# weitianxin/MACR

Hardware: AMD Instinct MI355X
Metric: train interactions/sec + eval users/sec (full-catalog top-K@20) (higher is better)
Workload: dtype f32; 1 GPU; gowalla-shape MACR-MF rubibceboth d=64 batch=4096 c=40 (n_users=29858, n_items=40981); synthetic Xavier tables, Zipf positives, batches as sampled (grouped on the device inside the step); parallelism=replicas x1 (train) / item-sharded x1 + RCCL all-gather (eval), global_batch=4096

## Files before the change

### macr_amd/csrc/train_kernels.hip

```cpp
#include "common.hpp"
#include "refsort.hpp"
#include "spmm.hpp"

#include <type_traits>

namespace macr {

#ifdef MACR_ABL_NOATOMIC
#define MACR_ATOMIC_ADD(p, v) (*(p) = (v))
#else
#define MACR_ATOMIC_ADD(p, v) unsafeAtomicAdd((p), (v))
#endif

constexpr int kPartStride = 4;

template <int LPR>
struct RowGroup {
    static constexpr int kRowsPerWave = kWave / LPR;
    static constexpr int kRowsPerBlock = 256 / LPR;
    int sub;
    int slot;
    __device__ RowGroup() {
        sub = threadIdx.x % LPR;
        slot = threadIdx.x / LPR;
// ... 383 lines not shown
    __shared__ float s_lr[kLazyRing];
    s_lr[threadIdx.x] = state->lr[threadIdx.x];
    const uint32_t T = state->t;
    __syncthreads();
    const int sub = threadIdx.x % LPR;
    for (long long k = blockIdx.x * (256LL / LPR) + threadIdx.x / LPR; k < n; k += gridDim.x * (256LL / LPR)) {
        const int row = rows[k];
        float4 x = make_float4(0, 0, 0, 0);
        if (row >= 0) x = lazy_row4<LPR>(tb, row, sub, T, s_lr, b1, b2, eps);
        st4(out + ((size_t)k * LPR + sub) * 4, x);
    }
}

constexpr float kBxbYHi = 6.0f, kBxbYLoPairs = -60.0f, kBxbYLoSingle = -20.0f;
constexpr float kBprZLoPairs = -40.0f;
constexpr int kNeutralTileMax = 8;

struct PendingAdam {
    const float *mU, *vU, *gU, *mI, *vI, *gI;
    int32_t *tU, *tI;
    const float *mw, *vw, *mwu, *vwu;
    const StepScalars *scal;
    float b1, b2, eps;
    const uint32_t *stU, *stI;
    const LazyState *lazy;
};

template <int LPR, int PENDING, bool RUBIBPR = false>
__global__ __launch_bounds__(256) void k_pair_fwd(
    int B, int Bp, const int32_t *__restrict__ u, const int32_t *__restrict__ i, const int32_t *__restrict__ j,
    const float *__restrict__ Usrc, const float *__restrict__ Isrc,
    const float *__restrict__ w, const float *__restrict__ wu,
    float *__restrict__ fwd, float *__restrict__ part, int reg_on_gathered, float *__restrict__ gw, PendingAdam pa,
    int user_branch, const float *__restrict__ Bsrc = nullptr) {
    constexpr int d = 4 * LPR;
    __shared__ float red[48];
    __shared__ float s_lr[PENDING == 2 ? kLazyRing : 1];
    RowGroup<LPR> g;
    const int t = blockIdx.x * RowGroup<LPR>::kRowsPerBlock + g.slot;
    float sq = 0.f, litem = 0.f, luser = 0.f;
    uint32_t T = 0;
    if (PENDING == 2) {
        s_lr[threadIdx.x] = pa.lazy->lr[threadIdx.x];
        T = pa.lazy->t;
        __syncthreads();
    }
    if (!PENDING && blockIdx.x == 0) {
        for (int k = threadIdx.x; k < kBranchSlots * 2 * d; k += 256) gw[k] = 0.f;
    }
    if (t < B) {
        const int ru = u[t], ri = i[t], rj = j[t];
        float4 eu = ld4(Usrc + (size_t)ru * d + 4 * g.sub);
        float4 ei = ld4(Isrc + (size_t)ri * d + 4 * g.sub);
        float4 ej = ld4(Isrc + (size_t)rj * d + 4 * g.sub);
        float4 w4 = ld4(w + 4 * g.sub), wu4 = ld4(wu + 4 * g.sub);
        if (PENDING) {
            const float lr_t = pa.scal->lr_t;
            const size_t au = (size_t)ru * d + 4 * g.sub, ai = (size_t)ri * d + 4 * g.sub, aj = (size_t)rj * d + 4 * g.sub;
            float4 mu = ld4(pa.mU + au), vu = ld4(pa.vU + au), mi = ld4(pa.mI + ai), vi = ld4(pa.vI + ai);
            float4 mj = ld4(pa.mI + aj), vj = ld4(pa.vI + aj);
            const float4 gu = ld4(pa.gU + au), gi = ld4(pa.gI + ai), gj = ld4(pa.gI + aj);
            float4 gw4 = make_float4(0, 0, 0, 0), gwu4 = make_float4(0, 0, 0, 0);
#pragma unroll
            for (int k = 0; k < kBranchSlots; ++k) {
                gw4 = add4(gw4, ld4(gw + (size_t)k * 2 * d + 4 * g.sub));
                gwu4 = add4(gwu4, ld4(gw + (size_t)k * 2 * d + d + 4 * g.sub));
            }
            float4 mw4 = ld4(pa.mw + 4 * g.sub), vw4 = ld4(pa.vw + 4 * g.sub);
            float4 mwu4 = ld4(pa.mwu + 4 * g.sub), vwu4 = ld4(pa.vwu + 4 * g.sub);
            if (PENDING == 2) {
                const uint32_t upto = T - 1u, su_ = pa.stU[ru], si_ = pa.stI[ri], sj_ = pa.stI[rj];
                if (g.sub == 0) {
// ... 31 lines not shown
            const float ssi = sigmoid_acc(si), ssj = sigmoid_acc(sj), ssu = user_branch ? sigmoid_acc(su) : 1.0f;
            fwd[0 * (size_t)Bp + t] = p;
            fwd[1 * (size_t)Bp + t] = n;
            fwd[2 * (size_t)Bp + t] = ssi * ssu;
            fwd[3 * (size_t)Bp + t] = ssj * ssu;
            fwd[4 * (size_t)Bp + t] = ssi;
            fwd[5 * (size_t)Bp + t] = ssj;
            if (RUBIBPR) {
                float hi, hj;
                litem = PairLossBPR::term(si, sj, 1.0f, hi, hj);
                fwd[6 * (size_t)Bp + t] = fabsf(hj);
            } else {
                fwd[6 * (size_t)Bp + t] = (p < -20.0f || n > kBxbYHi || n < kBxbYLoPairs) ? -ssu : ssu;
                litem = -logf(ssi + eps) + -logf((1.0f - ssj) + eps);
            }
            luser = user_branch ? -logf(ssu + eps) + -logf((1.0f - ssu) + eps) : 0.0f;
        }
    }
    float s0 = sq, s1 = litem, s2 = luser;
    block_sum3(s0, s1, s2, red);
    if (threadIdx.x == 0) {
        float *o = part + (size_t)blockIdx.x * kPartStride;
        o[0] = s0; o[1] = s1; o[2] = s2; o[3] = 0.f;
    }
}

struct BatchSort {
    const int32_t *u, *i, *j;
    int B;
    int rb0;
    int32_t *perm, *us, *is, *js;
    const float *outflag;
    int nneu, ncbx;
};

constexpr int kBucketSpan = 512;

template <int NW>
__device__ __forceinline__ void batch_bucket_block(const BatchSort &s, int part, uint32_t *s_hist ) {
    const int t = threadIdx.x, wid = t >> 6, lane = t & 63;
    const int plo = part * kBucketSpan, phi = plo + kBucketSpan < s.B ? plo + kBucketSpan : s.B;
    constexpr int per = kBucketSpan / NW;
    const int lo = plo + wid * per < phi ? plo + wid * per : phi, hi = lo + per < phi ? lo + per : phi;
    const uint32_t *keys = reinterpret_cast<const uint32_t *>(s.i);
    for (int k = t; k < NW * kRadix; k += NW * 64) s_hist[k] = 0;
    __syncthreads();
    wave_count(keys, lo, hi, 0, s_hist + wid * kRadix);
    __syncthreads();
    block_digit_offsets<NW>(s_hist, s_hist + NW * kRadix, nullptr, 0);
    uint32_t *offs = s_hist + wid * kRadix;
    const uint64_t below = (1ull << lane) - 1ull;
    constexpr int NQ = per / 64;
    int32_t ri[NQ], ru[NQ], rj[NQ];
    if (lo < hi) {
#pragma unroll
        for (int q = 0; q < NQ; ++q) {
            const int p = lo + q * 64 + lane, pc = p < hi ? p : hi - 1;
            ri[q] = s.i[pc]; ru[q] = s.u[pc]; rj[q] = s.j[pc];
        }
    }
#pragma unroll
    for (int q = 0; q < NQ; ++q) {
        if (lo + q * 64 >= hi) break;
        const int p = lo + q * 64 + lane;
        const bool valid = p < hi;
        const uint32_t dgt = (uint32_t)ri[q] & 255u;
// ... 54 lines not shown
                const float4 f4 = at < B ? ld4(sort.outflag + at + 4 * e) : make_float4(0, 0, 0, 0);
                bits |= ((__float_as_uint(f4.x) >> 31) | ((__float_as_uint(f4.y) >> 31) << 1) | ((__float_as_uint(f4.z) >> 31) << 2) |
                         ((__float_as_uint(f4.w) >> 31) << 3)) << (4 * e);
            }
            int mine = __popc(bits);
            const int pair2 = mine + __shfl_xor(mine, 1, 64);
            const int tile = pair2 + __shfl_xor(pair2, 2, 64);
            if (tile > kNeutralTileMax) mine = 0;
            for (uint64_t hit = __ballot(mine != 0); hit; hit &= hit - 1) {
                const int src = __builtin_ctzll(hit);
                for (uint32_t wv = (uint32_t)__builtin_amdgcn_readlane((int)bits, src); wv; wv &= wv - 1) {
                    const int mine_now = idx++ % nslot == slot;
                    if (!mine_now) continue;
                    const int cj = base + 16 * src + __builtin_ctz(wv);
                    const v2f pn = {p[cj], n[cj]};
                    v2f accj = {0.f, 0.f};
#pragma unroll
                    for (int q = 0; q < R; ++q) {
                        const v2f z = pn * (abn[q] * (-kLog2e));
                        const v2f dd = v2f{__builtin_amdgcn_exp2f(z.x), __builtin_amdgcn_exp2f(z.y)} + one;
                        const v2f sg = {__builtin_amdgcn_rcpf(dd.x), __builtin_amdgcn_rcpf(dd.y)};
                        const v2f om = one - sg;
                        const v2f ts = sg + eps, tom = om + eps;
                        const float txy = ts.x * tom.y;
                        l2n += __builtin_amdgcn_logf(txy);
                        const float r2 = __builtin_amdgcn_rcpf(txy);
                        const v2f h = (sg * om) * r2;
                        const v2f g = v2f{h.x * tom.y, h.y * ts.x};
                        dabn[q] = __builtin_elementwise_fma(g, pn, dabn[q]);
                        accj = __builtin_elementwise_fma(g, abn[q], accj);
                    }
                    const float sx = wave_sum(accj.x), sy = wave_sum(accj.y);
                    if (lane == 0) {
                        colpart[((size_t)rb * 2 + 0) * Bp + cj] = -sx;
                        colpart[((size_t)rb * 2 + 1) * Bp + cj] = sy;
                    }
                }
            }
        }
#pragma unroll
        for (int q = 0; q < R; ++q) {
            s_row[wid][0][q * 64 + lane] = -dabn[q].x;
            s_row[wid][1][q * 64 + lane] = dabn[q].y;
        }
        const float lsum = block_sum(-l2n * kLn2, red);
        if (t == 0) lpart[(size_t)rb * ncbx + ncb + part] = lsum;
        for (int e = t; e < 2 * RB; e += 256) {
            const int q = e / RB, rr = e % RB, r = rb * RB + rr;
            rowpart[((size_t)(ncb + part) * 2 + q) * Bp + r] = (s_row[0][q][rr] + s_row[1][q][rr]) + (s_row[2][q][rr] + s_row[3][q][rr]);
        }
        return;
    }
    if ((int)blockIdx.x >= nbxb + nbn && (int)blockIdx.x < nbxb + nbn + nsort) {
        __builtin_amdgcn_s_setprio(3);
#ifndef MACR_ABL_NOGROUP
        batch_bucket_block<4>(sort, blockIdx.x - nbxb - nbn, s_hist);
#endif
        return;
    }
    const bool is_adam = ADAM && (int)blockIdx.x >= nbxb + nbn + nsort;
    const int ablk = blockIdx.x - nbxb - nbn - nsort, bblk = blockIdx.x;
    if (is_adam) {
#ifndef MACR_ABL_ADAM_NOPRIO
        __builtin_amdgcn_s_setprio(3);
#endif
        if (ADAM == 2) adam_lazy_scan_block(adam, (long long)ablk, scal->lr_t, s_red);
        else adam_block<true>(adam, (long long)ablk, scal->lr_t, s_red);
        return;
    }
    const int cb = bblk % ncb, rb = sort.rb0 + bblk / ncb, t = threadIdx.x, lane = t & 63, wid = t >> 6;
    const float *p = fwd, *n = fwd + Bp, *a = fwd + 2 * (size_t)Bp, *b = fwd + 3 * (size_t)Bp;
    const float kLog2e = 1.4426950408889634f, kLn2 = 0.6931471805599453f;
    const v2f one = {1.0f, 1.0f}, eps = {1e-10f, 1e-10f};
    v2f ab[R], abs_[R], dab[R];
    bool rok[R];
#pragma unroll
    for (int q = 0; q < R; ++q) {
        const int r = rb * RB + q * 64 + lane;
        rok[q] = FULL || r < B;
        ab[q] = v2f{rok[q] ? a[r] : 0.f, rok[q] ? b[r] : 0.f};
        abs_[q] = ab[q] * (-kLog2e);
        dab[q] = v2f{0.f, 0.f};
// ... 180 lines not shown
#if defined(MACR_ABL_BXB_EXACT)
    const bool fast = false;
#elif defined(MACR_ABL_BXB_FORCEFAST)
    const bool fast = true;
#else
    float amax = 0.f, bmax = 0.f;
#pragma unroll
    for (int q = 0; q < R; ++q) { amax = fmaxf(amax, ab[q].x); bmax = fmaxf(bmax, ab[q].y); }
#pragma unroll
    for (int m = 1; m < 64; m <<= 1) { amax = fmaxf(amax, __shfl_xor(amax, m, 64)); bmax = fmaxf(bmax, __shfl_xor(bmax, m, 64)); }
    constexpr float YLO = R >= 2 ? kBxbYLoPairs : kBxbYLoSingle, YHI = kBxbYHi;
    const float xlo = cn.x * amax, yv = cn.y * bmax;
    bool out;
    if constexpr (CELL == kCellBpr) {
        bool nan_row = false;
#pragma unroll
        for (int q = 0; q < R; ++q) nan_row = nan_row || !(ab[q].x + ab[q].y == ab[q].x + ab[q].y);
        out = nan_row || !(fminf(xlo, 0.f) - fmaxf(yv, 0.f) >= kBprZLoPairs) || !(cn.x == cn.x) || !(cn.y == cn.y);
    } else {
        out = !(xlo >= -20.0f) || !(yv >= YLO) || !(yv <= YHI) || !(amax <= 1.0f) || !(bmax <= 1.0f);
    }
    const bool fast = !__any(out);
#endif
    if constexpr (CELL == kCellBpr) {
        if constexpr (R == 1) run_tile_bpr(std::true_type{});
        else if (fast) run_tile_bpr(std::true_type{});
        else run_tile_bpr(std::false_type{});
    } else if (fast) {
        if constexpr (R >= 2) run_tile_pairs(); else run_tile(std::true_type{});
    } else {
        run_tile(std::false_type{});
    }
    if (FULL && sort.nneu) l2.x += 2.0f * (float)(R * (int)__popcll(__ballot(own_out)));
    if (cok && !own_out) {
        colpart[((size_t)rb * 2 + 0) * Bp + c] = -acc.x;
        colpart[((size_t)rb * 2 + 1) * Bp + c] = acc.y;
    }
#pragma unroll
    for (int q = 0; q < R; ++q) {
        s_row[wid][0][q * 64 + lane] = -dab[q].x;
        s_row[wid][1][q * 64 + lane] = dab[q].y;
    }
    const float lsum = block_sum(-(l2.x + l2.y) * kLn2, red);
    if (t == 0) lpart[(size_t)rb * ncbx + cb] = lsum;
    for (int e = t; e < 2 * RB; e += 256) {
        const int q = e / RB, rr = e % RB, r = rb * RB + rr;
        if (FULL || r < B)
            rowpart[((size_t)cb * 2 + q) * Bp + r] = (s_row[0][q][rr] + s_row[1][q][rr]) + (s_row[2][q][rr] + s_row[3][q][rr]);
    }
}

constexpr int kChunkT = 16;

template <int D>
struct WaveRow {
    static constexpr int EPL = (D + 63) / 64;
    static constexpr int kActive = D < 64 ? D : 64;
};

template <int D, bool EGO = false>
__device__ __forceinline__ void combine_positive_rows(const int *s_pos, const float (*s_gi)[D], float *gI,
                                                      int32_t *cnt = nullptr, const float *s_sb = nullptr, float *sbr = nullptr) {
    constexpr int NP = D >= 256 ? 1 : 256 / D;
    const int k = threadIdx.x % D, part = threadIdx.x / D;
    int rows[kChunkT];
#pragma unroll
    for (int s = 0; s < kChunkT; ++s) rows[s] = s_pos[s];
#pragma unroll
    for (int L = 0; L < kChunkT; ++L) {
        if (rows[L] < 0 || (L % NP) != part) continue;
        bool first = true;
#pragma unroll
        for (int s0 = 0; s0 < L; ++s0) first = first && rows[s0] != rows[L];
        if (!first) continue;
        float acc = s_gi[L][k], sb = EGO ? s_sb[L] : 0.f;
        int mult = 1;
#pragma unroll
        for (int s2 = L + 1; s2 < kChunkT; ++s2)
            if (rows[s2] == rows[L]) { acc += s_gi[s2][k]; ++mult; if (EGO) sb += s_sb[s2]; }
        MACR_ATOMIC_ADD(gI + (size_t)rows[L] * D + k, acc);
        if (cnt && k == 0) atomicAdd(cnt + rows[L], mult);
        if (EGO && k == 0) MACR_ATOMIC_ADD(sbr + rows[L], sb);
    }
}

template <int D, bool EGO = false, bool RUBIBPR = false>
__global__ __launch_bounds__(256) void k_pair_bwd(
    int B, int Bp, int nrb, int ncb, const int32_t *__restrict__ perm, const int32_t *__restrict__ u,
    const int32_t *__restrict__ i, const int32_t *__restrict__ j, const float *__restrict__ Usrc,
    const float *__restrict__ Isrc,
    const float *__restrict__ w, const float *__restrict__ wu, const float *__restrict__ fwd,
    const float *__restrict__ rowpart, const float *__restrict__ colpart,
    float *gU, float *gI, int32_t *touchedU, int32_t *touchedI, float *__restrict__ wpart,
    float alpha, float beta, float coef, float *adam_pow, StepScalars *scal, float lr, float b1, float b2,
    LossArgs L, int32_t *cnt_pos, LazyState *lazy = nullptr, int nneu = 0, const float *__restrict__ Bsrc = nullptr,
    float *sbr = nullptr) {
    constexpr int EPL = WaveRow<D>::EPL;
    __shared__ float s_w[4][2][D];
    __shared__ float s_gi[kChunkT][D];
    __shared__ int s_pos[kChunkT];
    __shared__ float s_sb[EGO ? kChunkT : 1];
    const int nblk = gridDim.x - 1;
    if ((int)blockIdx.x == nblk) {
        if (threadIdx.x == 0) {
            const float p1 = adam_pow[0], p2 = adam_pow[1];
            const float lr_t = lr * sqrtf(1.0f - p2) / (1.0f - p1);
            scal->lr_t = lr_t;
            adam_pow[0] = p1 * b1;
            adam_pow[1] = p2 * b2;
            if (lazy) lazy_tick(lazy, lr_t);
        }
        if (L.losses && threadIdx.x < 64) finalize_losses(L, threadIdx.x);
        return;
    }
    const int lane = threadIdx.x & 63, wid = threadIdx.x >> 6;
    const bool act = lane < WaveRow<D>::kActive;
    float wk[EPL], wuk[EPL], aw[EPL], awu[EPL];
#pragma unroll
    for (int e = 0; e < EPL; ++e) {
        const int k = lane + 64 * e;
        wk[e] = act ? w[k] : 0.f; wuk[e] = act ? wu[k] : 0.f; aw[e] = 0.f; awu[e] = 0.f;
    }
    const float inv_b2 = 1.0f / ((float)B * (float)B), eps = 1e-10f, invB = 1.0f / (float)B;
    constexpr int SPW = kChunkT / 4;
    for (int chunk = blockIdx.x; chunk * kChunkT < B; chunk += nblk) {
        const int slot0 = chunk * kChunkT + wid * SPW;
        int my_idx = 0;
        {
            const int tq = slot0 + (lane % SPW);
            if (lane < 4 * SPW && tq < B) my_idx = (lane < SPW ? u : lane < 2 * SPW ? i : lane < 3 * SPW ? j : perm)[tq];
        }
        float reu[SPW][EPL], rei[SPW][EPL], rej[SPW][EPL];
        float rbi[EGO ? SPW : 1][EPL], rbj[EGO ? SPW : 1][EPL];
        int rru[SPW], rri[SPW], rrj[SPW];
#pragma unroll
        for (int q = 0; q < SPW; ++q) {
            rru[q] = __shfl(my_idx, q, kWave); rri[q] = __shfl(my_idx, SPW + q, kWave); rrj[q] = __shfl(my_idx, 2 * SPW + q, kWave);
#pragma unroll
            for (int e = 0; e < EPL; ++e) {
                const int k = act ? lane + 64 * e : 0;
                reu[q][e] = Usrc[(size_t)rru[q] * D + k]; rei[q][e] = Isrc[(size_t)rri[q] * D + k]; rej[q][e] = Isrc[(size_t)rrj[q] * D + k];
                if (EGO) { rbi[q][e] = Bsrc[(size_t)rri[q] * D + k]; rbj[q][e] = Bsrc[(size_t)rrj[q] * D + k]; }
            }
        }
        const int q_own = lane >> 4, kk = lane & 15;
        float dp = 0.f, dn = 0.f, da = 0.f, db = 0.f, ssi = 0.f, ssj = 0.f, ssu = 0.f;
        const bool own_ok = slot0 + q_own < B;
        const int t_own = own_ok ? __shfl(my_idx, 3 * SPW + q_own, kWave) : 0;
        {
            float cp[4], cn[4], ra[2], rb[2];
#pragma unroll
            for (int m = 0; m < 4; ++m) {
                const int k = kk + 16 * m, kc = k < nrb ? k : 0;
                cp[m] = colpart[((size_t)kc * 2) * Bp + t_own]; cn[m] = colpart[((size_t)kc * 2 + 1) * Bp + t_own];
            }
#pragma unroll
            for (int m = 0; m < 2; ++m) {
                const int k = kk + 16 * m, kc = k < ncb ? k : 0;
                ra[m] = rowpart[((size_t)kc * 2) * Bp + t_own]; rb[m] = rowpart[((size_t)kc * 2 + 1) * Bp + t_own];
            }
            const int kn = kk < nneu ? ncb + kk : 0;
            const float dan = rowpart[((size_t)kn * 2) * Bp + t_own], dbn = rowpart[((size_t)kn * 2 + 1) * Bp + t_own];
            const float sg = fabsf(fwd[(4 + (kk < 3 ? kk : 0)) * (size_t)Bp + t_own]);
#pragma unroll
            for (int m = 0; m < 4; ++m) { const bool ok = own_ok && kk + 16 * m < nrb; dp += ok ? cp[m] : 0.f; dn += ok ? cn[m] : 0.f; }
#pragma unroll
            for (int m = 0; m < 2; ++m) { const bool ok = own_ok && kk + 16 * m < ncb; da += ok ? ra[m] : 0.f; db += ok ? rb[m] : 0.f; }
            const bool neu_ok = own_ok && kk < nneu;
            da += neu_ok ? dan : 0.f; db += neu_ok ? dbn : 0.f;
            ssi = (own_ok && kk < 3) ? sg : 0.f;
            if (own_ok) {
                for (int k = kk + 64; k < nrb; k += 16) { dp += colpart[((size_t)k * 2) * Bp + t_own]; dn += colpart[((size_t)k * 2 + 1) * Bp + t_own]; }
                for (int k = kk + 32; k < ncb; k += 16) { da += rowpart[((size_t)k * 2) * Bp + t_own]; db += rowpart[((size_t)k * 2 + 1) * Bp + t_own]; }
            }
        }
#pragma unroll
        for (int m = 1; m < 16; m <<= 1) {
            dp += __shfl_xor(dp, m, kWave); dn += __shfl_xor(dn, m, kWave);
            da += __shfl_xor(da, m, kWave); db += __shfl_xor(db, m, kWave);
        }
        ssj = __shfl(ssi, (lane & 48) + 1, kWave); ssu = __shfl(ssi, (lane & 48) + 2, kWave); ssi = __shfl(ssi, lane & 48, kWave);
        dp *= inv_b2; dn *= inv_b2; da *= inv_b2; db *= inv_b2;
        const float hbpr = ssu;
        if (RUBIBPR) ssu = 1.0f;
        const float dsi_own = da * (ssi * (1.0f - ssi)) * ssu + (alpha * invB) * (RUBIBPR ? -hbpr : dneglog_sig(ssi, eps));
        const float dsj_own = db * (ssj * (1.0f - ssj)) * ssu + (alpha * invB) * (RUBIBPR ? hbpr : dneglog_1msig(ssj, eps));
        const float dsu_own = (da * ssi + db * ssj) * (ssu * (1.0f - ssu)) +
                              (beta * invB) * (dneglog_sig(ssu, eps) + dneglog_1msig(ssu, eps));
#pragma unroll
        for (int q = 0; q < SPW; ++q) {
            const int slot = wid * SPW + q;
            if (slot0 + q >= B) { if (lane == 0) s_pos[slot] = -1; continue; }
            const float dpq = __shfl(dp, q * 16, kWave), dnq = __shfl(dn, q * 16, kWave);
            const float dsi = __shfl(dsi_own, q * 16, kWave), dsj = __shfl(dsj_own, q * 16, kWave), dsu = __shfl(dsu_own, q * 16, kWave);
            const int ru = rru[q], ri = rri[q], rj = rrj[q];
            if (act) {
#pragma unroll
                for (int e = 0; e < EPL; ++e) {
                    const int k = lane + 64 * e;
                    const float eu = reu[q][e], ei = rei[q][e], ej = rej[q][e];
                    const float gu = fmaf(coef, eu, fmaf(dsu, wuk[e], fmaf(dnq, ej, dpq * ei)));
                    const float gi = EGO ? fmaf(coef, ei, dpq * eu) : fmaf(coef, ei, fmaf(dsi, wk[e], dpq * eu));
                    const float gj = EGO ? fmaf(coef, ej, dnq * eu) : fmaf(coef, ej, fmaf(dsj, wk[e], dnq * eu));
                    MACR_ATOMIC_ADD(gU + (size_t)ru * D + k, gu);
                    MACR_ATOMIC_ADD(gI + (size_t)rj * D + k, gj);
                    s_gi[slot][k] = gi;
                    if (EGO) aw[e] = fmaf(dsi, rbi[EGO ? q : 0][e], fmaf(dsj, rbj[EGO ? q : 0][e], aw[e]));
                    else aw[e] = fmaf(dsi, ei, fmaf(dsj, ej, aw[e]));
                    awu[e] = fmaf(dsu, eu, awu[e]);
                }
            }
            if (lane == 0) {
// ... 662 lines not shown
#ifdef MACR_BXB_ROWS
    return MACR_BXB_ROWS;
#endif
    static const int forced = getenv("MACR_BXB_ROWS") ? atoi(getenv("MACR_BXB_ROWS")) : 0;
    if (forced == 1 || forced == 2 || forced == 4) return forced;
    if (B >= 4096) return 4;
    return 1;
}

static inline bool use_staging(int B) {
    static const char *env = getenv("MACR_STAGING");
    if (env && (env[0] == '0' || env[0] == '1')) return env[0] == '1';
    return B > kSmallBatchMax;
}

struct PairWs {
    StepScalars *scal;
    float *gw;
    bool staged;
    int32_t *perm, *us, *is, *js;
    uint32_t *ska, *sva, *skb, *svb;
    uint32_t *ghist;
    uint32_t *n_work;
    float *stage;
    int nblk_bwd;
    float *fwd;
    float *part;
    float *part2;
    float *lpart;
    float *rowpart;
    float *colpart;
    int Bp, nrb, ncb, rows, nblk_pair;
    int nneu, ncbx;
    float *cpart;
    float *wblk;
    float *spart;
    size_t bytes;
};

static PairWs carve_pair_ws(void *base, int B, int d, bool force_staged = false, bool neutral = true) {
    PairWs w;
    const int lpr = d / 4, rpb = 256 / lpr;
    w.Bp = (int)align_up((size_t)B, 256);
    w.rows = bxb_rows(B);
    w.nrb = w.Bp / (64 * w.rows);
    w.ncb = w.Bp / 256;
    static const bool no_neutral = getenv("MACR_BXB_NEUTRAL") && getenv("MACR_BXB_NEUTRAL")[0] == '0';
    w.nneu = (!force_staged && B % 256 == 0 && !no_neutral && neutral) ? 1 : 0;
    w.ncbx = w.ncb + w.nneu;
    w.nblk_pair = (B + rpb - 1) / rpb;
    w.staged = force_staged || use_staging(B);
    if (w.staged) w.nblk_bwd = w.nblk_pair < 4096 ? w.nblk_pair : 4096;
    else w.nblk_bwd = (B + kChunkT - 1) / kChunkT < 1024 ? (B + kChunkT - 1) / kChunkT : 1024;
    char *p = static_cast<char *>(base);
    size_t off = 0;
    auto take = [&](size_t bytes) { void *r = p ? p + off : nullptr; off += align_up(bytes, 256); return r; };
    w.scal = static_cast<StepScalars *>(take(sizeof(StepScalars)));
    w.gw = static_cast<float *>(take((size_t)kBranchSlots * 2 * d * 4));
    w.fwd = static_cast<float *>(take((size_t)7 * w.Bp * 4));
    const int nblk_loss = (B + kChunkT - 1) / kChunkT < 1024 ? (B + kChunkT - 1) / kChunkT : 1024;
    int npart = w.nblk_pair > w.nblk_bwd ? w.nblk_pair : w.nblk_bwd;
    npart = npart > nblk_loss ? npart : nblk_loss;
    w.part = static_cast<float *>(take((size_t)npart * kPartStride * 4));
    w.part2 = static_cast<float *>(take((size_t)npart * kPartStride * 4));
    w.lpart = static_cast<float *>(take((size_t)w.nrb * w.ncbx * 4));
    w.rowpart = static_cast<float *>(take((size_t)w.ncbx * 2 * w.Bp * 4));
    w.colpart = static_cast<float *>(take((size_t)w.nrb * 2 * w.Bp * 4));
    const size_t nsort = 3 * (size_t)B;
    w.ska = w.sva = w.skb = w.svb = nullptr;
    w.perm = w.us = w.is = w.js = nullptr; w.ghist = nullptr; w.stage = nullptr; w.n_work = nullptr;
    w.cpart = w.wblk = w.spart = nullptr;
    if (w.staged) {
        w.ska = static_cast<uint32_t *>(take(nsort * 4)); w.sva = static_cast<uint32_t *>(take(nsort * 4));
        w.skb = static_cast<uint32_t *>(take(nsort * 4)); w.svb = static_cast<uint32_t *>(take(nsort * 4));
        w.ghist = static_cast<uint32_t *>(take(sort_hist_words((int)nsort) * 4));
        w.n_work = static_cast<uint32_t *>(take(4));
        w.stage = static_cast<float *>(take(nsort * d * 4));
    } else {
        w.perm = static_cast<int32_t *>(take((size_t)B * 4)); w.us = static_cast<int32_t *>(take((size_t)B * 4));
        w.is = static_cast<int32_t *>(take((size_t)B * 4));   w.js = static_cast<int32_t *>(take((size_t)B * 4));
    }
    w.bytes = off;
    return w;
}

static PairWs carve_pair_ws_det(void *base, int B, int d) {
    PairWs w = carve_pair_ws(base, B, d, true, false);
    const int ch = d / 4 < 16 ? d / 4 : 16;
    char *p = static_cast<char *>(base);
    auto take = [&](size_t bytes) { void *r = p ? p + w.bytes : nullptr; w.bytes += align_up(bytes, 256); return r; };
    w.cpart = static_cast<float *>(take(2 * ((3 * (size_t)B + ch - 1) / ch) * d * 4));
    w.wblk = static_cast<float *>(take((size_t)w.nblk_bwd * 2 * d * 4));
    return w;
}

template <int CELL = kCellBce>
static void launch_bxb_rows(const PairWs &ws, int B, int nbxb, const AdamArgs *pending, long long n_adam_blocks,
                            const BatchSort &sort, hipStream_t st) {
    const int nsort = (sort.B + kBucketSpan - 1) / kBucketSpan + sort.nneu * ws.nrb;
    const bool full = B % 256 == 0;
#ifdef MACR_ABL_XNOADAM
    n_adam_blocks = 0;
#endif
    auto launch = [&](auto rows) {
        constexpr int R = decltype(rows)::value;
        if (pending && pending->lazy) {
            const unsigned grid = (unsigned)(nbxb + nsort + n_adam_blocks);
            if (full) k_bxb<R, true, 2, CELL><<<grid, 256, 0, st>>>(B, ws.Bp, ws.ncb, nbxb, ws.fwd, ws.rowpart, ws.colpart, ws.lpart, *pending, ws.scal, sort);
            else      k_bxb<R, false, 2, CELL><<<grid, 256, 0, st>>>(B, ws.Bp, ws.ncb, nbxb, ws.fwd, ws.rowpart, ws.colpart, ws.lpart, *pending, ws.scal, sort);
        } else if (pending) {
            const unsigned grid = (unsigned)(nbxb + nsort + n_adam_blocks);
            if (full) k_bxb<R, true, 1, CELL><<<grid, 256, 0, st>>>(B, ws.Bp, ws.ncb, nbxb, ws.fwd, ws.rowpart, ws.colpart, ws.lpart, *pending, ws.scal, sort);
            else      k_bxb<R, false, 1, CELL><<<grid, 256, 0, st>>>(B, ws.Bp, ws.ncb, nbxb, ws.fwd, ws.rowpart, ws.colpart, ws.lpart, *pending, ws.scal, sort);
        } else {
            AdamArgs none;
            none.n_seg = 0;
            if (full) k_bxb<R, true, 0, CELL><<<nbxb + nsort, 256, 0, st>>>(B, ws.Bp, ws.ncb, nbxb, ws.fwd, ws.rowpart, ws.colpart, ws.lpart, none, ws.scal, sort);
            else      k_bxb<R, false, 0, CELL><<<nbxb + nsort, 256, 0, st>>>(B, ws.Bp, ws.ncb, nbxb, ws.fwd, ws.rowpart, ws.colpart, ws.lpart, none, ws.scal, sort);
        }
    };
    switch (ws.rows) {
        case 1: launch(std::integral_constant<int, 1>()); break;
        case 2: launch(std::integral_constant<int, 2>()); break;
        default: launch(std::integral_constant<int, 4>()); break;
    }
}

static BatchSort batch_sort_args(const PairWs &ws, int B = 0, const int32_t *u = nullptr, const int32_t *i = nullptr,
                                 const int32_t *j = nullptr) {
    BatchSort s;
    s.u = u; s.i = i; s.j = j; s.B = B; s.rb0 = 0;
    s.perm = ws.perm; s.us = ws.us; s.is = ws.is; s.js = ws.js;
    s.outflag = nullptr; s.nneu = 0; s.ncbx = ws.ncb;
    return s;
}

struct RefSort { const uint32_t *sk, *sv; uint32_t *free_key, *free_val; };
static RefSort ref_sort_result(const PairWs &ws, int flip) {
    RefSort r;
    r.sk = flip ? ws.skb : ws.ska; r.sv = flip ? ws.svb : ws.sva;
    r.free_key = flip ? ws.ska : ws.skb; r.free_val = flip ? ws.sva : ws.svb;
    return r;
}
static RefSort launch_ref_sort(int B, int n_urows, int n_irows, const int32_t *u, const int32_t *i, const int32_t *j,
                               const PairWs &ws, hipStream_t st) {
    k_refs_init<<<(B + 255) / 256 < 2048 ? (B + 255) / 256 : 2048, 256, 0, st>>>(B, n_urows, u, i, j, ws.ska, ws.sva, ws.n_work);
    return ref_sort_result(ws, launch_radix_sort(ws.ska, ws.sva, ws.skb, ws.svb, 3 * B, (uint32_t)(n_urows + n_irows - 1), ws.ghist, st));
}
__global__ __launch_bounds__(256) void k_ref_place(int n, const uint32_t *__restrict__ sv, uint32_t *__restrict__ place) {
    for (int p = blockIdx.x * 256 + threadIdx.x; p < n; p += gridDim.x * 256) place[sv[p]] = (uint32_t)p;
}
static int launch_seg_index(int B, int d, int n_urows, int n_irows, const RefSort &r, bool listed, float *gU, float *gI,
                            int32_t *tU, int32_t *tI, const PairWs &ws, hipStream_t st) {
    const int n = 3 * B;
    k_seg_scan<<<(n + 255) / 256, 256, 0, st>>>(n, n_urows, (uint32_t)(n_urows + n_irows), r.sk, tU, tI, r.free_key, ws.n_work);
    MACR_CHECK_LAUNCH("seg_index", st);
    MACR_DISPATCH_LPR(d, (k_seg_sum<LPR><<<1024, 256, 0, st>>>(r.free_key, ws.n_work, n_urows, r.sk, listed ? nullptr : r.sv, ws.stage, gU, gI)));
    MACR_CHECK_LAUNCH("seg_sum", st);
    return MACR_OK;
}
static int launch_seg_reduce(int B, int d, int n_urows, int n_irows, const RefSort &r, float *gU, float *gI, int32_t *tU,
                             int32_t *tI, const float *sst, float *sbr, const PairWs &ws, hipStream_t st) {
    const int n = 3 * B;
    MACR_DISPATCH_LPR(d, (k_seg_reduce<LPR><<<(n + 256 / LPR - 1) / (256 / LPR), 256, 0, st>>>(
                             n, n_urows, (uint32_t)(n_urows + n_irows), r.sk, r.sv, ws.stage, gU, gI, tU, tI, sst, sbr)));
    MACR_CHECK_LAUNCH("seg_reduce", st);
// ... 29 lines not shown
                                  hipStream_t st) {
    const int B = c.B, d = c.d, n_urows = c.n_urows, n_irows = c.n_irows, n = 3 * B;
    float *sbr = sst ? c.sbr : nullptr;
    const RefSort r = launch_ref_sort(B, n_urows, n_irows, c.u, c.i, c.j, ws, st);
    MACR_CHECK_LAUNCH("ref_sort", st);
    if (c.sk_sorted) *c.sk_sorted = r.sk;
    if (sv_sorted) {
        *sv_sorted = r.sv;
        return launch_seg_index(B, d, n_urows, n_irows, r, false, c.gU, c.gI, c.tU, c.tI, ws, st);
    }
    if (ws.cpart) {
        MACR_REQUIRE(!sst || (sbr && ws.spart), MACR_E_UNSUPPORTED, "pair: this workspace has no slots for the ego branch scalars");
        MACR_DISPATCH_LPR(d, (k_seg_reduce<LPR, true><<<(n + 256 / LPR - 1) / (256 / LPR), 256, 0, st>>>(
                                 n, n_urows, (uint32_t)(n_urows + n_irows), r.sk, r.sv, ws.stage, c.gU, c.gI, c.tU, c.tI, sst, sbr, ws.cpart, ws.spart)));
        MACR_CHECK_LAUNCH("seg_reduce", st);
        MACR_DISPATCH_LPR(d, (k_seg_fold<LPR><<<(n + 256 / LPR - 1) / (256 / LPR), 256, 0, st>>>(
                                 n, n_urows, (uint32_t)(n_urows + n_irows), r.sk, ws.cpart, c.gU, c.gI, sst ? ws.spart : nullptr, sbr)));
        MACR_CHECK_LAUNCH("seg_fold", st);
        return MACR_OK;
    }
    return launch_seg_reduce(B, d, n_urows, n_irows, r, c.gU, c.gI, c.tU, c.tI, sst, sbr, ws, st);
}

static int launch_pair(const PairCall &c, const PairWs &ws, hipStream_t st) {
    const int kind = c.kind, B = c.B, d = c.d;
    const macr_hyper *hp = c.hp;
    const int user_branch = kind == MACR_LOSS_RUBIBCEBOTH;
    const int rubibpr = kind == MACR_LOSS_RUBIBPR;
    const bool ego = c.Bsrc != nullptr;
    MACR_REQUIRE(!rubibpr || (ws.nneu == 0 && !ego), MACR_E_INVALID, "pair: the BPR cell has no neutral blocks and no ego branch");
    BatchSort sort = batch_sort_args(ws, B, c.u, c.i, c.j);
    if (ws.staged || c.loss_only) sort.B = 0;
    sort.outflag = ws.fwd + 6 * (size_t)ws.Bp; sort.nneu = ws.nneu; sort.ncbx = ws.ncbx;
    if (is_pair_loss(kind) && c.loss_only) {
        const int nb = (B + kChunkT - 1) / kChunkT < 1024 ? (B + kChunkT - 1) / kChunkT : 1024;
        float *const no_rows = nullptr;
        int32_t *const no_flags = nullptr;
        MACR_DISPATCH_PAIR_LOSS(kind, MACR_DISPATCH_D(d, (k_pair_normal<PL, D><<<nb, 256, 0, st>>>(
                                              B, c.u, c.i, c.j, c.Usrc, c.Isrc, no_rows, no_rows, no_flags, no_flags, ws.part, c.coef,
                                              c.reg_on_gathered, c.adam_pow, nullptr, ws.scal, hp->lr, hp->beta1, hp->beta2, nullptr))));
        MACR_CHECK_LAUNCH("pair_normal", st);
        return MACR_OK;
    }
    static const bool listed_ok = !(getenv("MACR_STAGE_LISTED") && atoi(getenv("MACR_STAGE_LISTED")) == 0);
    const bool listed = ws.staged && c.sv_sorted && listed_ok && !c.loss_only;
    RefSort rs = {};
    if (listed) {
        rs = launch_ref_sort(B, c.n_urows, c.n_irows, c.u, c.i, c.j, ws, st);
        MACR_CHECK_LAUNCH("ref_sort", st);
        k_ref_place<<<(3 * B + 255) / 256 < 4096 ? (3 * B + 255) / 256 : 4096, 256, 0, st>>>(3 * B, rs.sv, rs.free_val);
        MACR_CHECK_LAUNCH("ref_place", st);
        *c.sv_sorted = nullptr;
    }
    if (is_pair_loss(kind)) {
        if (ws.staged) {
            MACR_DISPATCH_PAIR_LOSS(kind, MACR_DISPATCH_LPR(d, (k_pair_normal_stage<PL, LPR><<<ws.nblk_bwd, 256, 0, st>>>(
                                              B, c.u, c.i, c.j, c.Usrc, c.Isrc, ws.stage, ws.part, c.coef, c.reg_on_gathered, c.adam_pow,
                                              c.adam_pow, ws.scal, hp->lr, hp->beta1, hp->beta2, listed ? rs.free_val : nullptr))));
            MACR_CHECK_LAUNCH("pair_normal", st);
            if (listed) return launch_seg_index(B, d, c.n_urows, c.n_irows, rs, true, c.gU, c.gI, c.tU, c.tI, ws, st);
            return launch_ref_sort_reduce(c, c.sv_sorted, nullptr, ws, st);
        }
        k_batch_sort<<<(B + kBucketSpan - 1) / kBucketSpan, 256, 0, st>>>(sort);
        MACR_CHECK_LAUNCH("batch_sort", st);
        MACR_DISPATCH_PAIR_LOSS(kind, MACR_DISPATCH_D(d, (k_pair_normal<PL, D><<<ws.nblk_bwd, 256, 0, st>>>(
                                              B, ws.us, ws.is, ws.js, c.Usrc, c.Isrc, c.gU, c.gI, c.tU, c.tI, ws.part, c.coef, c.reg_on_gathered,
                                              c.adam_pow, c.adam_pow, ws.scal, hp->lr, hp->beta1, hp->beta2, c.cnt_pos))));
        MACR_CHECK_LAUNCH("pair_normal", st);
        return MACR_OK;
    }
#define MACR_DISPATCH_RUBIBPR(...)                                          \
    if (rubibpr) { constexpr bool RB = true; __VA_ARGS__; } else { constexpr bool RB = false; __VA_ARGS__; }
    if (c.pa && c.pa->lazy) {
        MACR_DISPATCH_RUBIBPR(MACR_DISPATCH_LPR(d, (k_pair_fwd<LPR, 2, RB><<<ws.nblk_pair, 256, 0, st>>>(B, ws.Bp, c.u, c.i, c.j, c.Usrc, c.Isrc, c.w, c.wu, ws.fwd,
                                                                                            ws.part, c.reg_on_gathered, ws.gw, *c.pa, user_branch))));
    } else if (c.pa) {
        MACR_DISPATCH_RUBIBPR(MACR_DISPATCH_LPR(d, (k_pair_fwd<LPR, 1, RB><<<ws.nblk_pair, 256, 0, st>>>(B, ws.Bp, c.u, c.i, c.j, c.Usrc, c.Isrc, c.w, c.wu, ws.fwd,
                                                                                            ws.part, c.reg_on_gathered, ws.gw, *c.pa, user_branch))));
    } else {
        PendingAdam none = {};
        MACR_DISPATCH_RUBIBPR(MACR_DISPATCH_LPR(d, (k_pair_fwd<LPR, 0, RB><<<ws.nblk_pair, 256, 0, st>>>(B, ws.Bp, c.u, c.i, c.j, c.Usrc, c.Isrc, c.w, c.wu, ws.fwd,
                                                                                            ws.part, c.reg_on_gathered, ws.gw, none, user_branch, c.Bsrc))));
    }
    MACR_CHECK_LAUNCH("pair_fwd", st);
    MACR_DISPATCH_RUBIBPR(launch_bxb_rows<RB ? kCellBpr : kCellBce>(ws, B, ws.nrb * ws.ncb, c.pending, c.n_pending_blocks, sort, st));
    MACR_CHECK_LAUNCH(c.pending ? "bxb+adam" : "bxb", st);
    if (c.loss_only) return MACR_OK;
    LossArgs L;
    if (c.finalize) L = *c.finalize; else L.losses = nullptr;
    if (ws.staged) {
        const bool det = ws.wblk != nullptr;
        if (det) MACR_REQUIRE(!listed, MACR_E_UNSUPPORTED, "pair: the deterministic step is unfused");
        if (ego) MACR_REQUIRE(!listed, MACR_E_UNSUPPORTED, "pair: the ego branch has no indexed staging");
        float *sst = ego ? ws.fwd + 2 * (size_t)ws.Bp - B : nullptr;
        float *wpart = det ? ws.wblk : ws.gw;
#define MACR_PAIR_BWD_STAGE(EGO, RB, DET)                                                                                             \
        MACR_DISPATCH_LPR(d, (k_pair_bwd_stage<LPR, EGO, RB, DET><<<ws.nblk_bwd + 1, 256, 0, st>>>(                                   \
                                 B, ws.Bp, ws.nrb, ws.ncb, c.u, c.i, c.j, c.Usrc, c.Isrc, c.w, c.wu, ws.fwd, ws.rowpart, ws.colpart,  \
                                 ws.stage, wpart, hp->alpha, hp->beta, c.coef, c.adam_pow, ws.scal, hp->lr, hp->beta1, hp->beta2, L,  \
                                 listed ? rs.free_val : nullptr, 0, c.tick, ws.nneu, c.Bsrc, sst)))
        if (ego && det) { MACR_PAIR_BWD_STAGE(true, false, true); }
        else if (ego) { MACR_PAIR_BWD_STAGE(true, false, false); }
        else if (det) { MACR_DISPATCH_RUBIBPR(MACR_PAIR_BWD_STAGE(false, RB, true)); }
        else { MACR_DISPATCH_RUBIBPR(MACR_PAIR_BWD_STAGE(false, RB, false)); }
#undef MACR_PAIR_BWD_STAGE
        MACR_CHECK_LAUNCH("pair_bwd", st);
        if (det) {
            k_branch_fold<<<(kBranchSlots * 2 * d + 255) / 256, 256, 0, st>>>(ws.nblk_bwd, 2 * d, ws.wblk, ws.gw);
            MACR_CHECK_LAUNCH("branch_fold", st);
        }
        if (listed) return launch_seg_index(B, d, c.n_urows, c.n_irows, rs, true, c.gU, c.gI, c.tU, c.tI, ws, st);
        return launch_ref_sort_reduce(c, det || ego ? nullptr : c.sv_sorted, sst, ws, st);
    }
    if (ego) {
        MACR_DISPATCH_D(d, (k_pair_bwd<D, true><<<ws.nblk_bwd + 1, 256, 0, st>>>(B, ws.Bp, ws.nrb, ws.ncb, ws.perm, ws.us, ws.is, ws.js,
                                                                            c.Usrc, c.Isrc, c.w, c.wu, ws.fwd, ws.rowpart, ws.colpart, c.gU,
                                                                            c.gI, c.tU, c.tI, ws.gw, hp->alpha, hp->beta, c.coef, c.adam_pow,
                                                                            ws.scal, hp->lr, hp->beta1, hp->beta2, L, c.cnt_pos, c.tick,
                                                                            ws.nneu, c.Bsrc, c.sbr)));
    } else {
        MACR_DISPATCH_RUBIBPR(MACR_DISPATCH_D(d, (k_pair_bwd<D, false, RB><<<ws.nblk_bwd + 1, 256, 0, st>>>(
                                 B, ws.Bp, ws.nrb, ws.ncb, ws.perm, ws.us, ws.is, ws.js, c.Usrc, c.Isrc, c.w, c.wu, ws.fwd, ws.rowpart, ws.colpart, c.gU,
                                 c.gI, c.tU, c.tI, ws.gw, hp->alpha, hp->beta, c.coef, c.adam_pow, ws.scal, hp->lr, hp->beta1, hp->beta2, L, c.cnt_pos,
                                 c.tick, ws.nneu))));
    }
#undef MACR_DISPATCH_RUBIBPR
    MACR_CHECK_LAUNCH("pair_bwd", st);
    return MACR_OK;
}

static void add_seg(AdamArgs &a, float *theta, float *m, float *v, float *g, int32_t *touched, long long rows,
                    long long &next_block, int n_parts = 0, int part_stride = 0) {
    AdamSeg &s = a.seg[a.n_seg++];
    s.theta = theta; s.m = m; s.v = v; s.g = g; s.touched = touched; s.stamp = nullptr;
    s.sv = nullptr; s.stage = nullptr;
    s.n_parts = n_parts; s.part_stride = part_stride;
    s.n_vec = rows * a.lpr;
    s.first_block = next_block;
    next_block += (s.n_vec + kAdamVecPerBlock - 1) / kAdamVecPerBlock;
}

static void adam_args_begin(AdamArgs &a, int d, const macr_hyper *hp) {
    a.n_seg = 0;
    a.lpr = d / 4; a.lpr_shift = d == 32 ? 3 : d == 64 ? 4 : d == 128 ? 5 : 6;
    a.b1 = hp->beta1; a.b2 = hp->beta2; a.eps = hp->adam_eps;
}
static void add_branch_segs(AdamArgs &a, int loss_kind, int d, float *w, float *mw, float *vw, float *wu, float *mwu, float *vwu,
                            float *gw, long long &nb) {
    if (!is_pair_loss(loss_kind)) add_seg(a, w, mw, vw, gw, nullptr, 1, nb, kBranchSlots, 2 * d);
    if (loss_kind == MACR_LOSS_RUBIBCEBOTH) add_seg(a, wu, mwu, vwu, gw + d, nullptr, 1, nb, kBranchSlots, 2 * d);
}
static LossArgs loss_args(int kind, int B, const macr_hyper *hp, float *losses) {
    LossArgs L;
    L.kind = kind; L.B = B; L.batch_size_cfg = hp->batch_size_cfg;
    L.alpha = hp->alpha; L.beta = hp->beta; L.decay = hp->decay; L.losses = losses;
    return L;
}

// ... 1096 lines not shown
```

Baseline: 122.0 million interactions/s.

## Accumulate batch-by-batch row/column partials via atomics into compact sums buffer

Adds a 4×Bp sums buffer that the forward kernel zeroes. The batch-by-batch tile kernels then add their row and column partial gradients into it atomically instead of writing per-block rowpart/colpart slabs. The backward kernel reads four precomputed sums per row, replacing the strided loops over all column-block partials and the cross-lane shuffle reduction. This trades a large partial-buffer write/read pass for atomic contention and non-deterministic summation order. It is enabled by default when B is a multiple of 256 and no lazy/tick path is used, with an env var to disable it.

New measurement: 122.1 million interactions/s, median of 2. No clear change (+0.1%).

```diff
diff --git a/macr_amd/csrc/train_kernels.hip b/macr_amd/csrc/train_kernels.hip
--- a/macr_amd/csrc/train_kernels.hip
+++ b/macr_amd/csrc/train_kernels.hip
@@ -439,12 +439,13 @@
     const float *__restrict__ Usrc, const float *__restrict__ Isrc,
     const float *__restrict__ w, const float *__restrict__ wu,
     float *__restrict__ fwd, float *__restrict__ part, int reg_on_gathered, float *__restrict__ gw, PendingAdam pa,
-    int user_branch, const float *__restrict__ Bsrc = nullptr) {
+    int user_branch, const float *__restrict__ Bsrc = nullptr, float *__restrict__ sums = nullptr) {
     constexpr int d = 4 * LPR;
     __shared__ float red[48];
     __shared__ float s_lr[PENDING == 2 ? kLazyRing : 1];
     RowGroup<LPR> g;
     const int t = blockIdx.x * RowGroup<LPR>::kRowsPerBlock + g.slot;
+    if (sums && g.sub < 4 && t < Bp) sums[(size_t)g.sub * Bp + t] = 0.f;
     float sq = 0.f, litem = 0.f, luser = 0.f;
     uint32_t T = 0;
     if (PENDING == 2) {
@@ -542,6 +543,7 @@
     int32_t *perm, *us, *is, *js;
     const float *outflag;
     int nneu, ncbx;
+    float *sums;
 };
 
 constexpr int kBucketSpan = 512;
@@ -662,8 +664,13 @@
                     }
                     const float sx = wave_sum(accj.x), sy = wave_sum(accj.y);
                     if (lane == 0) {
-                        colpart[((size_t)rb * 2 + 0) * Bp + cj] = -sx;
-                        colpart[((size_t)rb * 2 + 1) * Bp + cj] = sy;
+                        if (sort.sums) {
+                            unsafeAtomicAdd(sort.sums + cj, -sx);
+                            unsafeAtomicAdd(sort.sums + (size_t)Bp + cj, sy);
+                        } else {
+                            colpart[((size_t)rb * 2 + 0) * Bp + cj] = -sx;
+                            colpart[((size_t)rb * 2 + 1) * Bp + cj] = sy;
+                        }
                     }
                 }
             }
@@ -677,7 +684,9 @@
         if (t == 0) lpart[(size_t)rb * ncbx + ncb + part] = lsum;
         for (int e = t; e < 2 * RB; e += 256) {
             const int q = e / RB, rr = e % RB, r = rb * RB + rr;
-            rowpart[((size_t)(ncb + part) * 2 + q) * Bp + r] = (s_row[0][q][rr] + s_row[1][q][rr]) + (s_row[2][q][rr] + s_row[3][q][rr]);
+            const float rs = (s_row[0][q][rr] + s_row[1][q][rr]) + (s_row[2][q][rr] + s_row[3][q][rr]);
+            if (!sort.sums) rowpart[((size_t)(ncb + part) * 2 + q) * Bp + r] = rs;
+            else if (rs != 0.f) unsafeAtomicAdd(sort.sums + (size_t)(2 + q) * Bp + r, rs);
         }
         return;
     }
@@ -924,7 +933,12 @@
         run_tile(std::false_type{});
     }
     if (FULL && sort.nneu) l2.x += 2.0f * (float)(R * (int)__popcll(__ballot(own_out)));
-    if (cok && !own_out) {
+    if (sort.sums) {
+        if (cok && !own_out) {
+            unsafeAtomicAdd(sort.sums + c, -acc.x);
+            unsafeAtomicAdd(sort.sums + (size_t)Bp + c, acc.y);
+        }
+    } else if (cok && !own_out) {
         colpart[((size_t)rb * 2 + 0) * Bp + c] = -acc.x;
         colpart[((size_t)rb * 2 + 1) * Bp + c] = acc.y;
     }
@@ -937,8 +951,11 @@
     if (t == 0) lpart[(size_t)rb * ncbx + cb] = lsum;
     for (int e = t; e < 2 * RB; e += 256) {
         const int q = e / RB, rr = e % RB, r = rb * RB + rr;
-        if (FULL || r < B)
-            rowpart[((size_t)cb * 2 + q) * Bp + r] = (s_row[0][q][rr] + s_row[1][q][rr]) + (s_row[2][q][rr] + s_row[3][q][rr]);
+        if (FULL || r < B) {
+            const float rs = (s_row[0][q][rr] + s_row[1][q][rr]) + (s_row[2][q][rr] + s_row[3][q][rr]);
+            if (sort.sums) unsafeAtomicAdd(sort.sums + (size_t)(2 + q) * Bp + r, rs);
+            else rowpart[((size_t)cb * 2 + q) * Bp + r] = rs;
+        }
     }
 }
 
@@ -976,7 +993,7 @@
     }
 }
 
-template <int D, bool EGO = false, bool RUBIBPR = false>
+template <int D, bool EGO = false, bool RUBIBPR = false, bool SUMS = false>
 __global__ __launch_bounds__(256) void k_pair_bwd(
     int B, int Bp, int nrb, int ncb, const int32_t *__restrict__ perm, const int32_t *__restrict__ u,
     const int32_t *__restrict__ i, const int32_t *__restrict__ j, const float *__restrict__ Usrc,
@@ -986,7 +1003,7 @@
     float *gU, float *gI, int32_t *touchedU, int32_t *touchedI, float *__restrict__ wpart,
     float alpha, float beta, float coef, float *adam_pow, StepScalars *scal, float lr, float b1, float b2,
     LossArgs L, int32_t *cnt_pos, LazyState *lazy = nullptr, int nneu = 0, const float *__restrict__ Bsrc = nullptr,
-    float *sbr = nullptr) {
+    float *sbr = nullptr, const float *__restrict__ sums = nullptr) {
     constexpr int EPL = WaveRow<D>::EPL;
     __shared__ float s_w[4][2][D];
     __shared__ float s_gi[kChunkT][D];
@@ -1039,7 +1056,14 @@
         float dp = 0.f, dn = 0.f, da = 0.f, db = 0.f, ssi = 0.f, ssj = 0.f, ssu = 0.f;
         const bool own_ok = slot0 + q_own < B;
         const int t_own = own_ok ? __shfl(my_idx, 3 * SPW + q_own, kWave) : 0;
-        {
+        if (SUMS) {
+            const float sv = sums[(size_t)(kk & 3) * Bp + t_own];
+            const float sg = fabsf(fwd[(4 + (kk < 3 ? kk : 0)) * (size_t)Bp + t_own]);
+            const float s4 = own_ok ? sv : 0.f;
+            ssi = (own_ok && kk < 3) ? sg : 0.f;
+            dp = __shfl(s4, lane & 48, kWave); dn = __shfl(s4, (lane & 48) + 1, kWave);
+            da = __shfl(s4, (lane & 48) + 2, kWave); db = __shfl(s4, (lane & 48) + 3, kWave);
+        } else {
             float cp[4], cn[4], ra[2], rb[2];
 #pragma unroll
             for (int m = 0; m < 4; ++m) {
@@ -1066,10 +1090,12 @@
                 for (int k = kk + 32; k < ncb; k += 16) { da += rowpart[((size_t)k * 2) * Bp + t_own]; db += rowpart[((size_t)k * 2 + 1) * Bp + t_own]; }
             }
         }
-#pragma unroll
-        for (int m = 1; m < 16; m <<= 1) {
-            dp += __shfl_xor(dp, m, kWave); dn += __shfl_xor(dn, m, kWave);
-            da += __shfl_xor(da, m, kWave); db += __shfl_xor(db, m, kWave);
+        if (!SUMS) {
+#pragma unroll
+            for (int m = 1; m < 16; m <<= 1) {
+                dp += __shfl_xor(dp, m, kWave); dn += __shfl_xor(dn, m, kWave);
+                da += __shfl_xor(da, m, kWave); db += __shfl_xor(db, m, kWave);
+            }
         }
         ssj = __shfl(ssi, (lane & 48) + 1, kWave); ssu = __shfl(ssi, (lane & 48) + 2, kWave); ssi = __shfl(ssi, lane & 48, kWave);
         dp *= inv_b2; dn *= inv_b2; da *= inv_b2; db *= inv_b2;
@@ -1798,6 +1824,7 @@
     float *colpart;
     int Bp, nrb, ncb, rows, nblk_pair;
     int nneu, ncbx;
+    float *sums;
     float *cpart;
     float *wblk;
     float *spart;
@@ -1836,6 +1863,7 @@
     w.ska = w.sva = w.skb = w.svb = nullptr;
     w.perm = w.us = w.is = w.js = nullptr; w.ghist = nullptr; w.stage = nullptr; w.n_work = nullptr;
     w.cpart = w.wblk = w.spart = nullptr;
+    w.sums = nullptr;
     if (w.staged) {
         w.ska = static_cast<uint32_t *>(take(nsort * 4)); w.sva = static_cast<uint32_t *>(take(nsort * 4));
         w.skb = static_cast<uint32_t *>(take(nsort * 4)); w.svb = static_cast<uint32_t *>(take(nsort * 4));
@@ -1845,6 +1873,10 @@
     } else {
         w.perm = static_cast<int32_t *>(take((size_t)B * 4)); w.us = static_cast<int32_t *>(take((size_t)B * 4));
         w.is = static_cast<int32_t *>(take((size_t)B * 4));   w.js = static_cast<int32_t *>(take((size_t)B * 4));
+        const char *env_sums = getenv("MACR_BXB_SUMS");
+        const bool no_sums = env_sums && env_sums[0] == '0';
+        float *sums = static_cast<float *>(take((size_t)4 * w.Bp * 4));
+        if (B % 256 == 0 && !no_sums) w.sums = sums;
     }
     w.bytes = off;
     return w;
@@ -1897,7 +1929,7 @@
     BatchSort s;
     s.u = u; s.i = i; s.j = j; s.B = B; s.rb0 = 0;
     s.perm = ws.perm; s.us = ws.us; s.is = ws.is; s.js = ws.js;
-    s.outflag = nullptr; s.nneu = 0; s.ncbx = ws.ncb;
+    s.outflag = nullptr; s.nneu = 0; s.ncbx = ws.ncb; s.sums = nullptr;
     return s;
 }
 
@@ -1993,6 +2025,8 @@
     BatchSort sort = batch_sort_args(ws, B, c.u, c.i, c.j);
     if (ws.staged || c.loss_only) sort.B = 0;
     sort.outflag = ws.fwd + 6 * (size_t)ws.Bp; sort.nneu = ws.nneu; sort.ncbx = ws.ncbx;
+    float *const sums = (c.tick || (c.pa && c.pa->lazy) || c.loss_only) ? nullptr : ws.sums;
+    sort.sums = sums;
     if (is_pair_loss(kind) && c.loss_only) {
         const int nb = (B + kChunkT - 1) / kChunkT < 1024 ? (B + kChunkT - 1) / kChunkT : 1024;
         float *const no_rows = nullptr;
@@ -2037,11 +2071,11 @@
                                                                                             ws.part, c.reg_on_gathered, ws.gw, *c.pa, user_branch))));
     } else if (c.pa) {
         MACR_DISPATCH_RUBIBPR(MACR_DISPATCH_LPR(d, (k_pair_fwd<LPR, 1, RB><<<ws.nblk_pair, 256, 0, st>>>(B, ws.Bp, c.u, c.i, c.j, c.Usrc, c.Isrc, c.w, c.wu, ws.fwd,
-                                                                                            ws.part, c.reg_on_gathered, ws.gw, *c.pa, user_branch))));
+                                                                                            ws.part, c.reg_on_gathered, ws.gw, *c.pa, user_branch, nullptr, sums))));
     } else {
         PendingAdam none = {};
         MACR_DISPATCH_RUBIBPR(MACR_DISPATCH_LPR(d, (k_pair_fwd<LPR, 0, RB><<<ws.nblk_pair, 256, 0, st>>>(B, ws.Bp, c.u, c.i, c.j, c.Usrc, c.Isrc, c.w, c.wu, ws.fwd,
-                                                                                            ws.part, c.reg_on_gathered, ws.gw, none, user_branch, c.Bsrc))));
+                                                                                            ws.part, c.reg_on_gathered, ws.gw, none, user_branch, c.Bsrc, sums))));
     }
     MACR_CHECK_LAUNCH("pair_fwd", st);
     MACR_DISPATCH_RUBIBPR(launch_bxb_rows<RB ? kCellBpr : kCellBce>(ws, B, ws.nrb * ws.ncb, c.pending, c.n_pending_blocks, sort, st));
@@ -2073,18 +2107,20 @@
         if (listed) return launch_seg_index(B, d, c.n_urows, c.n_irows, rs, true, c.gU, c.gI, c.tU, c.tI, ws, st);
         return launch_ref_sort_reduce(c, det || ego ? nullptr : c.sv_sorted, sst, ws, st);
     }
+#define MACR_DISPATCH_SUMS(...)                                             \
+    if (sums) { constexpr bool SM = true; __VA_ARGS__; } else { constexpr bool SM = false; __VA_ARGS__; }
     if (ego) {
-        MACR_DISPATCH_D(d, (k_pair_bwd<D, true><<<ws.nblk_bwd + 1, 256, 0, st>>>(B, ws.Bp, ws.nrb, ws.ncb, ws.perm, ws.us, ws.is, ws.js,
-                                                                            c.Usrc, c.Isrc, c.w, c.wu, ws.fwd, ws.rowpart, ws.colpart, c.gU,
-                                                                            c.gI, c.tU, c.tI, ws.gw, hp->alpha, hp->beta, c.coef, c.adam_pow,
-                                                                            ws.scal, hp->lr, hp->beta1, hp->beta2, L, c.cnt_pos, c.tick,
-                                                                            ws.nneu, c.Bsrc, c.sbr)));
-    } else {
-        MACR_DISPATCH_RUBIBPR(MACR_DISPATCH_D(d, (k_pair_bwd<D, false, RB><<<ws.nblk_bwd + 1, 256, 0, st>>>(
+        MACR_DISPATCH_SUMS(MACR_DISPATCH_D(d, (k_pair_bwd<D, true, false, SM><<<ws.nblk_bwd + 1, 256, 0, st>>>(
                                  B, ws.Bp, ws.nrb, ws.ncb, ws.perm, ws.us, ws.is, ws.js, c.Usrc, c.Isrc, c.w, c.wu, ws.fwd, ws.rowpart, ws.colpart, c.gU,
                                  c.gI, c.tU, c.tI, ws.gw, hp->alpha, hp->beta, c.coef, c.adam_pow, ws.scal, hp->lr, hp->beta1, hp->beta2, L, c.cnt_pos,
-                                 c.tick, ws.nneu))));
-    }
+                                 c.tick, ws.nneu, c.Bsrc, c.sbr, sums))));
+    } else {
+        MACR_DISPATCH_SUMS(MACR_DISPATCH_RUBIBPR(MACR_DISPATCH_D(d, (k_pair_bwd<D, false, RB, SM><<<ws.nblk_bwd + 1, 256, 0, st>>>(
+                                 B, ws.Bp, ws.nrb, ws.ncb, ws.perm, ws.us, ws.is, ws.js, c.Usrc, c.Isrc, c.w, c.wu, ws.fwd, ws.rowpart, ws.colpart, c.gU,
+                                 c.gI, c.tU, c.tI, ws.gw, hp->alpha, hp->beta, c.coef, c.adam_pow, ws.scal, hp->lr, hp->beta1, hp->beta2, L, c.cnt_pos,
+                                 c.tick, ws.nneu, nullptr, nullptr, sums)))));
+    }
+#undef MACR_DISPATCH_SUMS
 #undef MACR_DISPATCH_RUBIBPR
     MACR_CHECK_LAUNCH("pair_bwd", st);
     return MACR_OK;
```
